# nyrahealth/CrisperWhisper

Measured on AMD Instinct MI355X. Metric: aligned words/s (RTF alongside), CrisperWhisper large-v3 geometry, 30 s chunks, full mel->encoder->decoder->DTW->words path, higher is better.
Workload: dtype bf16

## Files before the change

crisperwhisper_amd/_native.py:

```python
from __future__ import annotations

import ctypes as C
import os

_HERE = os.path.dirname(os.path.abspath(__file__))
LIB_PATH = os.environ.get("CW_LIB_PATH") or os.path.join(_HERE, "libcrisperwhisper.so")

CW_DTYPE_F32, CW_DTYPE_BF16, CW_DTYPE_F16 = 0, 1, 2
N_SAMPLES, N_FRAMES, N_CTX = 480000, 3000, 1500
STAGES = ("mel", "encoder", "cross_kv", "decode", "timestamps")
ALIGN_HEADS_MAX_BYTES = 8 << 30


class NativeLibraryError(RuntimeError):
    pass


class ModelDesc(C.Structure):
    _fields_ = [(n, C.c_int32) for n in (
        "d_model", "n_heads", "ffn_dim", "enc_layers", "dec_layers", "n_mels", "vocab_size",
        "max_target_positions", "median_filter_width", "dtype", "max_batch", "n_align")] + [
        ("align_layers", C.POINTER(C.c_int32)), ("align_heads", C.POINTER(C.c_int32))]


# ... 136 lines not shown
    "cw_test_cross_attention": (_I, [_P, _I, _I, _I, _I, _P, _P, _P, _I, _P, _P, _P, _P]),
    "cw_test_cross_attention_fused": (_I, [_P, _I, _I, _I, _I, _P, _P, _P, _P, _P, _I, _P, _P, _I, _P, _P, _P, _P]),
    "cw_test_fold": (_I, [_P, C.POINTER(FoldArgs)]),
    "cw_test_gemv_stack": (_I, [_P, C.POINTER(GemvStackArgs)]),
    "cw_test_gemv_epi": (_I, [_P, C.POINTER(GemvEpiArgs)]),
    "cw_test_self_attention": (_I, [_P, _I, _I, _I, _I, _P, _P, _P, _P, _I, _P, _I, _I, _I, _I, _P, _P, _P]),
    "cw_test_beam_state": (_I, [_P, _I, _P, _P, _P]),
    "cw_test_prefill_gemm": (_I, [_P, _I, _I, _I, _I, _P, _P, _P, _P]),
    "cw_test_prefill_attention": (_I, [_P, _I, _I, _I, _I, _I, _I, _I, _P, _P, _P, _P]),
    "cw_test_prefill_align_attention": (_I, [_P, _I, _I, _I, _I, _I, _I, _P, _P, _P, _P, _P]),
    "cw_test_score_head": (_I, [_P, _I, _I, _I, _P, _P, _P, _P, _P, _P, _P, _P]),
    "cw_time_score_head": (_I, [_P, _I, _I, _I, _P]),
    "cw_test_beam_topk": (_I, [_P, _I, _P, _P, _I, _I, _I, _I, _P, _P]),
    "cw_test_beam_x": (_I, [_P, _I, _P]),
    "cw_test_sample": (_I, [_P, _I, _P, _P, _I, _I, _I, _I, _P]),
    "cw_test_sample_seeded": (_I, [_P, _I, _P, _P, _I, _I, _I, _I, C.c_float, C.c_uint64, _P, _P]),
    "cw_test_sample_logprobs": (_I, [_P, _I, _P, _P, _I, _I, _I, _I, C.c_float, C.c_uint64, _P, _P, _P, _P]),
    "cw_test_sample_top_logprobs": (_I, [_P, _I, _P, _P, _I, _I, _I, _I, C.c_float, C.c_uint64, _P, _P, _I, _P, _P, _P, _P]),
    "cw_test_sample_biased": (_I, [_P, _I, _P, _P, _I, _I, _I, _I, C.c_float, C.c_uint64, _P, _P, _I, _I, _P, _P, _P, _P, _P, _P, _P, _P]),
    "cw_stage_times": (_I, [_P, _P, _P, _I]),
    "cw_time_kernel": (_I, [_P, _I, _I, _I, _P, _P]),
    "cw_time_decode_stage": (_I, [_P, _I, _I, _I, _P, _P, _P, _P]),
    "cw_decode_stage_name": (C.c_char_p, [_I]),
    "cw_handoff_fallbacks": (_I, [_P]),
    "cw_handoff_resumes": (_I, [_P]),
    "cw_decode_stage_launches": (_I, [_P, _I]),
}

_lib = None

# ... 27 lines not shown
```

crisperwhisper_amd/csrc/elementwise.hip:

```cpp
#include "common.h"
#include "kernels.h"
#include <stdlib.h>

namespace CW_NS {

template <typename T>
__global__ __launch_bounds__(256) void layernorm_kernel(const float* __restrict__ x, const float* __restrict__ g,
                                                        const float* __restrict__ b, T* __restrict__ out, int rows,
                                                        int d) {
    const int lane = threadIdx.x & 63;
    const int row = blockIdx.x * 4 + (threadIdx.x >> 6);
    if (row >= rows) return;
    const float* xr = x + (size_t)row * d;
    T* o = out + (size_t)row * d;
    if (d <= 2048) {
        float4 v[8];
        float s = 0.f;
#pragma unroll
        for (int c = 0; c < 8; ++c) {
            const int k = (lane + 64 * c) * 4;
            v[c] = (k < d) ? *(const float4*)(xr + k) : make_float4(0.f, 0.f, 0.f, 0.f);
            s += (v[c].x + v[c].y) + (v[c].z + v[c].w);
        }
        const float mean = wave_sum(s) / (float)d;
// ... 196 lines not shown
    if (L < 1 || L > SB_MAX_LEN || L > t) return false;
    bool ok = true;
    for (int k = 0; k < L - 1; ++k) ok &= (ids[t - L + 1 + k] == tab[SB_TOK + o + k]);
    return ok;
}
__device__ inline float seq_bias_of(const int* __restrict__ tab, int tok, const int* __restrict__ ids, int t) {
    const int n = min(tab[SB_SLICE + SAMPLE_NS], SB_MAX_SEQ);
    int lo = 0, hi = n;
    while (lo < hi) { const int mid = (lo + hi) >> 1; if (tab[SB_LAST + mid] < tok) lo = mid + 1; else hi = mid; }
    float sum = 0.f;
    for (int e = lo; e < n && tab[SB_LAST + e] == tok; ++e)
        if (seq_bias_applies(tab, e, ids, t)) sum = __fadd_rn(sum, __int_as_float(tab[SB_VAL + e]));
    return sum;
}
#define SAMPLE_THREADS 256
template <bool TOPK, bool BIAS>
__global__ __launch_bounds__(256) void sample_partial_kernel(const float* __restrict__ logits, const int* ids_all, const int* cfg, const int* pos,
                                                             const int* last_ts_tok, const unsigned char* __restrict__ mask, int ldv, int ids_stride,
                                                             SampleParams p, SamplePart* __restrict__ part) {
    __shared__ float s_f[64];
    __shared__ int s_i[64];
    const int b = blockIdx.x, sl = blockIdx.y, tid = threadIdx.x, lane = tid & 63, wave = tid >> 6;
    const float* lg = logits + (size_t)b * ldv;
    const int* ids = ids_all + (size_t)b * ids_stride;
    const int n_prompt = cfg[0], min_new_tokens = cfg[1];
    const int t = pos[b] + 1, tb = p.timestamp_begin;
    const int n_gen = t - n_prompt;
    const bool last_ts = n_gen >= 1 && ids[t - 1] >= tb;
    const bool penult_ts = n_gen < 2 || ids[t - 2] >= tb;
    const int last_tok = last_ts_tok[b];
    const int ts_floor = (last_tok >= 0) ? ((last_ts && !penult_ts) ? last_tok : last_tok + 1) : tb;
    const bool at_begin = (n_gen == 0);
    const int ts_cap = (at_begin && p.max_initial_timestamp_index >= 0) ? tb + p.max_initial_timestamp_index : 0x7fffffff;
    const int per4 = ((ldv >> 2) + SAMPLE_NS - 1) / SAMPLE_NS;
    const int lo4 = sl * per4, hi4 = min(ldv >> 2, lo4 + per4);
    const float4* lg4 = (const float4*)lg;
    const uchar4* mk4 = (const uchar4*)mask;
    ArgPair bt = {-INFINITY, 0x7fffffff}, bs = {-INFINITY, 0x7fffffff};
    ArgPair pt = {-INFINITY, 0x7fffffff}, ps = {-INFINITY, 0x7fffffff};
    const float temp = p.samp ? __uint_as_float(p.samp[0]) : 0.f;
    const bool sampling = temp > 0.f;
    unsigned seed_lo = 0, seed_hi = 0, stream_lo = 0, stream_hi = 0;
    if (sampling) { seed_lo = p.samp[1]; seed_hi = p.samp[2]; stream_lo = p.samp[4 + 2 * b]; stream_hi = p.samp[5 + 2 * b]; }
    float sv[4][4]; int nmine = 0;
    float tv[4][4];
    float rm = -INFINITY, rs = 0.f;
    float rv[4][4];
    if (TOPK) {
#pragma unroll
        for (int it = 0; it < 4; ++it)
#pragma unroll
            for (int j = 0; j < 4; ++j) rv[it][j] = -INFINITY;
    }
    __shared__ float4 s_bias4[BIAS ? 1024 : 1];
    if constexpr (BIAS) {
        __shared__ int s_bl[SB_MAX_SEQ];
        __shared__ float s_bv[SB_MAX_SEQ];
        float* s_bias = (float*)s_bias4;
        for (int k = tid; k < per4; k += 256) s_bias4[k] = make_float4(0.f, 0.f, 0.f, 0.f);
        const int* tab = p.seq_bias;
        const int e0 = tab[SB_SLICE + sl], ne = min(tab[SB_SLICE + sl + 1] - e0, SB_MAX_SEQ);
        const bool have = tid < ne && e0 >= 0 && e0 + ne <= SB_MAX_SEQ;
        int mylast = -1;
        float myval = NAN;
        if (have) {
            mylast = tab[SB_LAST + e0 + tid];
            if (seq_bias_applies(tab, e0 + tid, ids, t)) myval = __int_as_float(tab[SB_VAL + e0 + tid]);
        }
        s_bl[tid] = mylast; s_bv[tid] = myval;
        __syncthreads();
        const int rel = mylast - lo4 * 4;
        if (have && rel >= 0 && rel < per4 * 4 && (tid == 0 || s_bl[tid - 1] != mylast)) {
            float sum = 0.f;
            for (int e = tid; e < SB_MAX_SEQ && s_bl[e] == mylast; ++e)
                if (s_bv[e] == s_bv[e]) sum = __fadd_rn(sum, s_bv[e]);
            s_bias[rel] = sum;
        }
        __syncthreads();
    }
    for (int i4 = lo4 + tid, it = 0; i4 < hi4; i4 += 256, ++it) {
        const float4 x = lg4[i4]; const uchar4 mk = mk4[i4];
        const float xs[4] = {x.x, x.y, x.z, x.w};
        float xe[4] = {x.x, x.y, x.z, x.w};
        if constexpr (BIAS) {
            const float4 bb = s_bias4[i4 - lo4];
            xe[0] = __fadd_rn(x.x, bb.x); xe[1] = __fadd_rn(x.y, bb.y); xe[2] = __fadd_rn(x.z, bb.z); xe[3] = __fadd_rn(x.w, bb.w);
        }
        const unsigned char ms[4] = {mk.x, mk.y, mk.z, mk.w};
        unsigned rnd[4] = {0u, 0u, 0u, 0u};
        if (sampling) philox4x32_10((unsigned)i4, (unsigned)t, stream_lo, stream_hi, seed_lo, seed_hi, rnd);
#pragma unroll
        for (int j = 0; j < 4; ++j) {
            const int v = i4 * 4 + j;
            float val = -INFINITY;
            if (v < p.V) {
                bool dead = (ms[j] & 1) || (at_begin && (ms[j] & 2));
                dead |= (v == p.eos && n_gen < min_new_tokens);
                if (last_ts) dead |= penult_ts ? (v >= tb) : (v < p.eos);
                dead |= (v >= tb && v < ts_floor);
                if (at_begin) dead |= (v < tb) || (v > ts_cap);
                if (!dead) val = xe[j];
                ArgPair c = {val, v};
                if (v < tb) bt = arg_better(bt, c); else bs = arg_better(bs, c);
                if (sampling && !dead) {
                    ArgPair q = {__fadd_rn(__fdiv_rn(val, temp), gumbel_from_bits(rnd[j])), v};
                    if (v < tb) pt = arg_better(pt, q); else ps = arg_better(ps, q);
                }
            }
            if (it < 4) { sv[it][j] = (v >= tb && v < p.V) ? val : -INFINITY; tv[it][j] = (v < tb) ? val : -INFINITY; }
            if (TOPK && it < 4) rv[it][j] = (v < p.V && xs[j] > -INFINITY) ? xs[j] : -INFINITY;
        }
        if (p.tok_lp) {
            float gm = -INFINITY;
#pragma unroll
            for (int j = 0; j < 4; ++j) if (i4 * 4 + j < p.V) gm = fmaxf(gm, xs[j]);
            if (gm > rm) { rs *= expf(rm - gm); rm = gm; }
            if (rm > -INFINITY) {
#pragma unroll
                for (int j = 0; j < 4; ++j) if (i4 * 4 + j < p.V) rs += expf(xs[j] - rm);
            }
        }
        nmine = it + 1;
    }
    bt = wave_argmax(bt);
    bs = wave_argmax(bs);
    if (lane == 0) { s_f[wave] = bt.v; s_i[wave] = bt.i; s_f[32 + wave] = bs.v; s_i[32 + wave] = bs.i; }
    __syncthreads();
    bt = {-INFINITY, 0x7fffffff}; bs = {-INFINITY, 0x7fffffff};
    for (int w = 0; w < 4; ++w) {
        bt = arg_better(bt, ArgPair{s_f[w], s_i[w]});
        bs = arg_better(bs, ArgPair{s_f[32 + w], s_i[32 + w]});
    }
    float acc = 0.f;
    if (bs.v > -INFINITY) {
        for (int it = 0; it < nmine && it < 4; ++it)
#pragma unroll
            for (int j = 0; j < 4; ++j) if (sv[it][j] > -INFINITY) acc += expf(sv[it][j] - bs.v);
    }
    __syncthreads();
    acc = block_sum(acc, s_f);
    float acc_t = 0.f;
    if (p.lp_sum) {
        if (bt.v > -INFINITY) {
            for (int it = 0; it < nmine && it < 4; ++it)
#pragma unroll
                for (int j = 0; j < 4; ++j) if (tv[it][j] > -INFINITY) acc_t += expf(tv[it][j] - bt.v);
        }
        __syncthreads();
        acc_t = block_sum(acc_t, s_f);
    }
    float raw_m = -INFINITY, raw_s = 0.f;
    if (p.tok_lp) {
        __syncthreads();
        raw_m = block_max(rm, s_f);
        __syncthreads();
        raw_s = block_sum(rm > -INFINITY ? rs * expf(rm - raw_m) : 0.f, s_f);
    }
    if (TOPK) {
        __shared__ float s_tf[8];
        __shared__ int s_ti[8];
        TopPair* rec = (TopPair*)p.top_part + ((size_t)b * SAMPLE_NS + sl) * CW_TOP_LOGPROBS_MAX;
        ArgPair prev = {INFINITY, -1};
        for (int r = 0; r < p.top_k; ++r) {
            ArgPair c = {-INFINITY, 0x7fffffff};
#pragma unroll
            for (int it = 0; it < 4; ++it)
#pragma unroll
                for (int j = 0; j < 4; ++j) {
                    const ArgPair q = {rv[it][j], (lo4 + tid + it * 256) * 4 + j};
                    if (q.v > -INFINITY && arg_after(q, prev)) c = arg_better(c, q);
                }
            c = wave_argmax(c);
            const int h = (r & 1) * 4;
            if (lane == 0) { s_tf[h + wave] = c.v; s_ti[h + wave] = c.i; }
            __syncthreads();
            c = {-INFINITY, 0x7fffffff};
            for (int w = 0; w < 4; ++w) c = arg_better(c, ArgPair{s_tf[h + w], s_ti[h + w]});
            if (tid == 0) { TopPair o; o.v = c.v; o.i = c.i; rec[r] = o; }
            prev = c;
        }
    }
// ... 18 lines not shown
        }
    }
    if (tid == 0) {
        SamplePart o; o.bt_v = bt.v; o.bt_i = bt.i; o.bs_v = bs.v; o.bs_i = bs.i; o.ts_sum = acc; o.pad[0] = acc_t; o.pad[1] = raw_m; o.pad[2] = raw_s;
        part[(size_t)b * SAMPLE_NS + sl] = o;
    }
}

template <typename T, bool TOPK, bool BIAS>
__global__ __launch_bounds__(1024) void sample_kernel(int* ids_all, const int* cfg, int* pos, int* finished, int* last_ts_tok,
                                                       const void* partials, int ids_stride, int timestamp_begin, SampleParams p) {
    __shared__ float s_f[64];
    __shared__ int s_i[64];
    __shared__ int s_tok;
    const int b = blockIdx.x, tid = threadIdx.x, lane = tid & 63, wave = tid >> 6, nw = SAMPLE_THREADS >> 6;
    const float* lg = p.logits + (size_t)b * p.ldv;
    int* ids = ids_all + (size_t)b * ids_stride;
    const int n_prompt = cfg[0], min_new_tokens = cfg[1], max_length = cfg[2], use_forced = cfg[3];
    const int t = pos[b] + 1, tb = timestamp_begin;
    const int n_gen = t - n_prompt;

    const int fin_in = finished[b];
    const bool was_finished = fin_in != 0;
    int forced = (p.forced && use_forced) ? p.forced[(size_t)b * ids_stride + t] : -1;

    const bool last_ts = n_gen >= 1 && ids[t - 1] >= tb;
    const bool penult_ts = n_gen < 2 || ids[t - 2] >= tb;
    const int last_tok = last_ts_tok[b];
    const int ts_floor = (last_tok >= 0) ? ((last_ts && !penult_ts) ? last_tok : last_tok + 1) : tb;
    const bool at_begin = (n_gen == 0);
    const int ts_cap = (at_begin && p.max_initial_timestamp_index >= 0) ? tb + p.max_initial_timestamp_index
                                                                         : 0x7fffffff;
    ArgPair bt = {-INFINITY, 0x7fffffff}, bs = {-INFINITY, 0x7fffffff};
    const SamplePart* pr = (const SamplePart*)partials + (size_t)b * SAMPLE_NS;
    for (int i = 0; i < SAMPLE_NS; ++i) {
        bt = arg_better(bt, ArgPair{pr[i].bt_v, pr[i].bt_i});
        bs = arg_better(bs, ArgPair{pr[i].bs_v, pr[i].bs_i});
    }
    const float M = fmaxf(bt.v, bs.v);
    float acc = 0.f;
    for (int i = 0; i < SAMPLE_NS; ++i)
        if (pr[i].bs_v > -INFINITY) acc += pr[i].ts_sum * expf(pr[i].bs_v - M);

    if (TOPK) {
        if (wave == 0 && !was_finished && n_gen >= 0) {
            float Mr = -INFINITY, Sr = 0.f;
            for (int i = 0; i < SAMPLE_NS; ++i) Mr = fmaxf(Mr, pr[i].pad[1]);
            for (int i = 0; i < SAMPLE_NS; ++i)
                if (pr[i].pad[1] > -INFINITY) Sr += pr[i].pad[2] * expf(pr[i].pad[1] - Mr);
            const float norm = Mr + logf(Sr);
            const TopPair* tp = (const TopPair*)p.top_part + (size_t)b * SAMPLE_NS * CW_TOP_LOGPROBS_MAX;
            const int k = p.top_k;
            const ArgPair none = {-INFINITY, 0x7fffffff};
            const bool have = (lane & (CW_TOP_LOGPROBS_MAX - 1)) < k;
            const ArgPair c0 = have ? ArgPair{tp[lane].v, tp[lane].i} : none;
            const ArgPair c1 = have ? ArgPair{tp[lane + 64].v, tp[lane + 64].i} : none;
            ArgPair prev = {INFINITY, -1}, mine = none;
            for (int r = 0; r < k; ++r) {
                ArgPair c = none;
                if (arg_after(c0, prev)) c = arg_better(c, c0);
                if (arg_after(c1, prev)) c = arg_better(c, c1);
                c = wave_argmax(c);
                if (lane == r) mine = c;
                prev = c;
            }
            if (lane < k) {
                const size_t o = ((size_t)b * ids_stride + t) * CW_TOP_LOGPROBS_MAX + lane;
                const bool ok = mine.v > -INFINITY;
                p.top_id[o] = ok ? mine.i : -1;
                p.top_lp[o] = ok ? mine.v - norm : NAN;
            }
        }
    }
    if (tid == 0) {
        bool force_ts = (acc > 0.f) && (logf(acc) > bt.v - M);
        int choice;
        if (force_ts || !(bt.v > -INFINITY)) choice = bs.i;
        else choice = arg_better(bt, bs).i;
        const float temp = p.samp ? __uint_as_float(p.samp[0]) : 0.f;
        if (temp > 0.f) {
            ArgPair pt = {-INFINITY, 0x7fffffff}, ps = {-INFINITY, 0x7fffffff};
            const SamplePert* pp = (const SamplePert*)p.pert + (size_t)b * SAMPLE_NS;
            for (int i = 0; i < SAMPLE_NS; ++i) {
                pt = arg_better(pt, ArgPair{pp[i].pt_v, pp[i].pt_i});
                ps = arg_better(ps, ArgPair{pp[i].ps_v, pp[i].ps_i});
            }
            choice = force_ts ? ps.i : arg_better(pt, ps).i;
        }
        if (!(M > -INFINITY) || choice < 0 || choice >= p.V) choice = 0;
        if (p.argmax_trace) p.argmax_trace[(size_t)b * ids_stride + t] = choice;
        int tok = (forced >= 0) ? forced : choice;
        if (p.lp_sum && !was_finished && n_gen >= 0) {
            float st = 0.f;
            for (int i = 0; i < SAMPLE_NS; ++i)
                if (pr[i].bt_v > -INFINITY) st += pr[i].pad[0] * expf(pr[i].bt_v - M);
            const float tot = acc + (force_ts ? 0.f : st);
            if (tot > 0.f && tok >= 0 && tok < p.V) {
                float xt = lg[tok];
                if constexpr (BIAS) xt = __fadd_rn(xt, seq_bias_of(p.seq_bias, tok, ids, t));
                p.lp_sum[b] += xt - (M + logf(tot));
                p.lp_cnt[b] += 1;
            }
        }
        if (p.tok_lp && !was_finished && n_gen >= 0 && tok >= 0 && tok < p.V) {
            float Mr = -INFINITY, Sr = 0.f;
            for (int i = 0; i < SAMPLE_NS; ++i) Mr = fmaxf(Mr, pr[i].pad[1]);
            for (int i = 0; i < SAMPLE_NS; ++i)
                if (pr[i].pad[1] > -INFINITY) Sr += pr[i].pad[2] * expf(pr[i].pad[1] - Mr);
            p.tok_lp[(size_t)b * ids_stride + t] = lg[tok] - (Mr + logf(Sr));
        }
        if (was_finished) tok = p.pad;
        if (fin_in != 2) ids[t] = tok;
        if (tok >= tb && n_gen >= 0) last_ts_tok[b] = tok;
        int fin = was_finished ? fin_in : ((n_gen >= 0 && tok == p.eos) || (t + 1 >= max_length));
        finished[b] = fin;
        if (!fin) atomicAdd(p.n_unfinished, 1);
        s_tok = tok;
        pos[b] = t;
    }
    __syncthreads();
    const int tok = s_tok;
    if (p.x_out && t < max_length) {
        const T* e = (const T*)p.embed + (size_t)tok * p.d;
        const float* pe = p.pos_embed + (size_t)t * p.d;
        for (int k = tid; k < p.d; k += SAMPLE_THREADS) {
            const float v = Act<T>::ld(e + k) + pe[k];
            p.x_out[(size_t)b * p.d + k] = sizeof(T) == 2 ? resid_grid(v) : v;
        }
    }
}

template <typename T>
__global__ __launch_bounds__(1024) void beam_topk_kernel(SampleParams p, int n_cand, float* __restrict__ cand_val,
                                                         int* __restrict__ cand_id) {
    __shared__ float s_f[64];
    __shared__ int s_i[64];
    const int b = blockIdx.x, tid = threadIdx.x, lane = tid & 63, wave = tid >> 6, nw = blockDim.x >> 6;
    const float* lg = p.logits + (size_t)b * p.ldv;
    const int* ids = p.ids + (size_t)b * p.ids_stride;
    const int n_prompt = p.cfg[0], min_new_tokens = p.cfg[1];
// ... 298 lines not shown
}

template <bool TOPK, bool BIAS>
static void launch_sample_t(const SampleParams& p, hipStream_t st) {
    hipLaunchKernelGGL((sample_partial_kernel<TOPK, BIAS>), dim3(p.B, SAMPLE_NS), dim3(256), 0, st, p.logits, (const int*)p.ids, p.cfg,
                       (const int*)p.pos, (const int*)p.last_ts_tok, p.mask, p.ldv, p.ids_stride, p, (SamplePart*)p.partials);
    if (p.embed_bf16)
        hipLaunchKernelGGL((sample_kernel<bf16_t, TOPK, BIAS>), dim3(p.B), dim3(SAMPLE_THREADS), 0, st, p.ids, p.cfg, p.pos, p.finished,
                           p.last_ts_tok, p.partials, p.ids_stride, p.timestamp_begin, p);
    else
        hipLaunchKernelGGL((sample_kernel<float, TOPK, BIAS>), dim3(p.B), dim3(SAMPLE_THREADS), 0, st, p.ids, p.cfg, p.pos, p.finished,
                           p.last_ts_tok, p.partials, p.ids_stride, p.timestamp_begin, p);
}
int cw_launch_sample(const SampleParams& p, hipStream_t st) {
    static_assert(SAMPLE_NS == 16 && SB_OFF > SB_SLICE + SAMPLE_NS, "the sequence_bias table holds one range per sampler slice");
    if (!p.partials || (p.ldv >> 2) > SAMPLE_NS * 1024 || (p.ldv & 3)) return CW_ERR_INVALID;
    const bool bias = p.seq_bias != nullptr;
    if (p.top_k != 0) {
        if (p.top_k < 0 || p.top_k > CW_TOP_LOGPROBS_MAX || !p.top_part || !p.top_id || !p.top_lp || !p.tok_lp) return CW_ERR_INVALID;
        if (bias) launch_sample_t<true, true>(p, st); else launch_sample_t<true, false>(p, st);
        return CW_OK;
    }
    if (bias) launch_sample_t<false, true>(p, st); else launch_sample_t<false, false>(p, st);
    return CW_OK;
}

}
```

crisperwhisper_amd/csrc/engine.hip:

```cpp
#include <chrono>
#include <hip/hip_runtime.h>
#include <stdarg.h>
#include <stdlib.h>
#include <string.h>
#include <set>
#include <string>
#include <vector>
#include <functional>
#include <algorithm>

#include "../../include/crisperwhisper.h"
#include "kernels.h"

static thread_local char g_err[512] = "";

#define KD(c, fn, ...) ((c)->f16 ? cw_f16::fn(__VA_ARGS__) : cw_bf16::fn(__VA_ARGS__))

#define CW_MAX_DEC_STAGES 24
enum DecStageKind { DST_OTHER = 0, DST_QKV_SELF, DST_QKV, DST_SELF_ATTN, DST_O_PROJ, DST_STACK, DST_STACK_CROSS, DST_CROSS_Q, DST_CROSS_ATTN,
                    DST_CROSS_O, DST_FC1, DST_FC2, DST_MLP_PAIR, DST_MLP_CHAIN, DST_N };
static const char* const kDecStageName[DST_N] = {
    "other (A/B path)", "LayerNorm + q/k/v projection + self-attention (qkv_self_kernel)", "LayerNorm + q/k/v projection + cache append",
    "self-attention", "self-attention out-projection", "fused out-projection + cross-query stage (gemv_stack_kernel)",
    "fused stage + cross-attention (dec_layer_a_kernel)", "LayerNorm + cross-attention query projection", "cross-attention",
// ... 4639 lines not shown
    if (er != hipSuccess) return fail(c, CW_ERR_HIP, "test_beam_topk: %s", hipGetErrorString(er));
    HIPCHK(c, hipMemcpy(cand_val, c->d_cand_val, (size_t)Bm * 64 * 4, hipMemcpyDeviceToHost));
    HIPCHK(c, hipMemcpy(cand_id, c->d_cand_id, (size_t)Bm * 64 * 4, hipMemcpyDeviceToHost));
    return CW_OK;
}

int32_t cw_test_beam_x(cw_ctx* c, int32_t rows, float* x) {
    if (rows < 1 || rows > c->Bm || !x) return fail(c, CW_ERR_INVALID, "test_beam_x: rows=%d", rows);
    HIPCHK(c, hipStreamSynchronize(c->st));
    HIPCHK(c, hipMemcpy(x, c->dx, (size_t)rows * c->d.d_model * 4, hipMemcpyDeviceToHost));
    return CW_OK;
}

static int test_sample(cw_ctx* c, int32_t nb, const float* logits, const int32_t* ids, int32_t t, int32_t n_prompt,
                       int32_t min_new_tokens, int32_t max_length, int32_t* choice_out, const int32_t* forced_tok = nullptr,
                       float* lp_out = nullptr, int32_t* top_id_out = nullptr, float* top_lp_out = nullptr);
int32_t cw_test_sample(cw_ctx* c, int32_t nb, const float* logits, const int32_t* ids, int32_t t, int32_t n_prompt,
                       int32_t min_new_tokens, int32_t max_length, int32_t* choice_out) {
    return test_sample(c, nb, logits, ids, t, n_prompt, min_new_tokens, max_length, choice_out);
}
int32_t cw_test_sample_seeded(cw_ctx* c, int32_t nb, const float* logits, const int32_t* ids, int32_t t, int32_t n_prompt,
                              int32_t min_new_tokens, int32_t max_length, float temperature, uint64_t seed,
                              const uint64_t* row_streams, int32_t* choice_out) {
    if (!logits || !ids || !choice_out) return fail(c, CW_ERR_INVALID, "test_sample_seeded: null argument");
    if (nb < 1 || nb > c->Bm || nb > 64) return fail(c, CW_ERR_INVALID, "test_sample_seeded: nb=%d outside 1 .. %d", nb, c->Bm < 64 ? c->Bm : 64);
    if (max_length <= n_prompt || max_length > c->d.max_target_positions || min_new_tokens < 0)
        return fail(c, CW_ERR_INVALID, "test_sample_seeded: max_length=%d / min_new_tokens=%d out of range", max_length, min_new_tokens);
    if (temperature > 0.f && !row_streams) return fail(c, CW_ERR_INVALID, "test_sample_seeded: a positive temperature needs row_streams");
    const std::vector<unsigned int> keep = c->samp_host;
    CWCHK(c, write_sampling(c, temperature, seed, row_streams, nb, "test_sample_seeded"));
    const int r = test_sample(c, nb, logits, ids, t, n_prompt, min_new_tokens, max_length, choice_out);
    HIPCHK(c, hipStreamSynchronize(c->st));
    HIPCHK(c, hipMemcpy(c->d_samp, keep.data(), keep.size() * 4, hipMemcpyHostToDevice));
    c->samp_host = keep;
// ... 66 lines not shown
    HIPCHK(c, hipMemset(c->d_lp_cnt, 0, (size_t)c->Bm * 4));
    const int r = cw_test_sample_top_logprobs(c, nb, logits, ids, t, n_prompt, min_new_tokens, max_length, temperature, seed, row_streams,
                                              forced_tok, k, choice_out, lp_out, top_id_out, top_lp_out);
    c->score_tokens = keep_score;
    int r2 = CW_OK;
    if (r == CW_OK) {
        hipError_t e = hipMemcpy(proc_lp_out, c->d_lp_sum, (size_t)nb * 4, hipMemcpyDeviceToHost);
        if (e != hipSuccess) r2 = fail(c, CW_ERR_HIP, "test_sample_biased: %s", hipGetErrorString(e));
    }
    drop_step_graphs(c);
    CWCHK(c, seq_bias_install(c, keep, keep_n));
    return r != CW_OK ? r : r2;
}
static int test_sample(cw_ctx* c, int32_t nb, const float* logits, const int32_t* ids, int32_t t, int32_t n_prompt,
                       int32_t min_new_tokens, int32_t max_length, int32_t* choice_out, const int32_t* forced_tok, float* lp_out,
                       int32_t* top_id_out, float* top_lp_out) {
    const int V = c->d.vocab_size, TGT = c->d.max_target_positions;
    if (!c->gen_set) return fail(c, CW_ERR_STATE, "cw_set_generation not called");
    if (nb < 1 || nb > c->Bm || t < n_prompt || t < 1 || t >= TGT || n_prompt < 1) return fail(c, CW_ERR_INVALID, "test_sample: bad args");
    const int tb = c->gen.no_timestamps_token_id + 1;
    std::vector<int> hid((size_t)nb * TGT, c->gen.pad_token_id), last(nb, -1), posv(64, t - 1);
    for (int b = 0; b < nb; ++b)
        for (int k = 0; k < t; ++k) {
            const int tok = ids[(size_t)b * t + k];
            if (tok < 0 || tok >= V) return fail(c, CW_ERR_INVALID, "test_sample: token %d out of range", tok);
            hid[(size_t)b * TGT + k] = tok;
            if (k >= n_prompt && tok >= tb) last[b] = tok;
        }
    HIPCHK(c, hipMemcpy(c->d_ids, hid.data(), hid.size() * 4, hipMemcpyHostToDevice));
    HIPCHK(c, hipMemcpy(c->d_last_ts, last.data(), nb * 4, hipMemcpyHostToDevice));
    HIPCHK(c, hipMemcpy(c->d_pos, posv.data(), 64 * 4, hipMemcpyHostToDevice));
    HIPCHK(c, hipMemset(c->d_finished, 0, nb * 4));
    HIPCHK(c, hipMemset(c->d_argmax, 0xff, (size_t)nb * TGT * 4));
    if (forced_tok) {
        std::vector<int> fr((size_t)nb * TGT, -1);
        for (int b = 0; b < nb; ++b) fr[(size_t)b * TGT + t] = forced_tok[b];
        HIPCHK(c, hipMemcpy(c->d_forced, fr.data(), fr.size() * 4, hipMemcpyHostToDevice));
    }
    if (lp_out) HIPCHK(c, hipMemset(c->d_tok_lp, 0xff, (size_t)nb * TGT * 4));
    if (top_id_out) {
        HIPCHK(c, hipMemset(c->d_top_id, 0xff, (size_t)nb * TGT * CW_TOP_LOGPROBS_MAX * 4));
        HIPCHK(c, hipMemset(c->d_top_lp, 0xff, (size_t)nb * TGT * CW_TOP_LOGPROBS_MAX * 4));
    }
    const int cfg[4] = {n_prompt, min_new_tokens, max_length, forced_tok ? 1 : 0};
    HIPCHK(c, hipMemcpy(c->d_cfg, cfg, sizeof(cfg), hipMemcpyHostToDevice));
    HIPCHK(c, hipMemcpy2D(c->dlogits, (size_t)c->Vpad * 4, logits, (size_t)V * 4, (size_t)V * 4, nb, hipMemcpyHostToDevice));
    const int n_padcol = c->Vpad - V;
// ... 197 lines not shown
```

crisperwhisper_amd/engine.py:

```python
from __future__ import annotations

import ctypes as C
import dataclasses
from typing import Dict, List, Optional, Sequence

import numpy as np

from . import _native as N

_GemvEpiArgs = N.GemvEpiArgs


def _ptr(a: Optional[np.ndarray]):
    return None if a is None else a.ctypes.data_as(C.c_void_p)


def _i32(x) -> np.ndarray:
    return np.ascontiguousarray(np.asarray(x, dtype=np.int32))


@dataclasses.dataclass
class ModelSpec:
    d_model: int
    n_heads: int
# ... 921 lines not shown
    def test_beam_x(self, rows: int) -> np.ndarray:
        x = np.zeros((int(rows), self.spec.d_model), np.float32)
        self._chk(self.lib.cw_test_beam_x(self.ctx, int(rows), _ptr(x)))
        return x

    def test_sample(self, logits: np.ndarray, ids: np.ndarray, n_prompt: int, min_new_tokens: int = 0,
                    max_length: Optional[int] = None) -> np.ndarray:
        lg = np.ascontiguousarray(logits, np.float32)
        ids = _i32(ids)
        nb, t = ids.shape
        out = np.zeros(nb, np.int32)
        self._chk(self.lib.cw_test_sample(self.ctx, nb, _ptr(lg), _ptr(ids), t, int(n_prompt), int(min_new_tokens),
                                          int(max_length or self.spec.max_target_positions), _ptr(out)))
        return out

    def test_sample_seeded(self, logits: np.ndarray, ids: np.ndarray, n_prompt: int, temperature: float, seed: int,
                           row_streams, min_new_tokens: int = 0, max_length: Optional[int] = None) -> np.ndarray:
        lg = np.ascontiguousarray(logits, np.float32)
        ids = _i32(ids)
        nb, t = ids.shape
        if lg.shape != (nb, self.spec.vocab_size):
            raise ValueError(f"logits must be [{nb}][{self.spec.vocab_size}], got {lg.shape}")
        rs = None if row_streams is None else np.ascontiguousarray(row_streams, dtype=np.uint64)
        if rs is not None and rs.shape != (nb,):
            raise ValueError(f"row_streams must hold one id per row ({nb}), got shape {rs.shape}")
        out = np.zeros(nb, np.int32)
        self._chk(self.lib.cw_test_sample_seeded(self.ctx, nb, _ptr(lg), _ptr(ids), t, int(n_prompt), int(min_new_tokens),
                                                 int(max_length or self.spec.max_target_positions), float(temperature),
                                                 int(seed) & (2 ** 64 - 1), _ptr(rs), _ptr(out)))
        return out
# ... 102 lines not shown
```

include/crisperwhisper.h:

```cpp
#ifndef CRISPERWHISPER_H
#define CRISPERWHISPER_H

#include <stdint.h>

#ifdef __cplusplus
extern "C" {
#endif

typedef struct cw_ctx cw_ctx;

#define CW_DTYPE_F32 0
#define CW_DTYPE_BF16 1
#define CW_DTYPE_F16 2

#define CW_N_SAMPLES 480000
#define CW_N_FRAMES 3000
#define CW_N_CTX 1500

typedef struct {
    int32_t d_model, n_heads, ffn_dim, enc_layers, dec_layers, n_mels, vocab_size;
    int32_t max_target_positions;
    int32_t median_filter_width;
    int32_t dtype;
    int32_t max_batch;
// ... 277 lines not shown
    float* cvec;
    int32_t* nt;
    int32_t* frag_tail_ok;
} cw_test_gemv_epi_args;
int32_t cw_test_gemv_epi(cw_ctx* ctx, const cw_test_gemv_epi_args* args);
int32_t cw_test_self_attention(cw_ctx* ctx, int32_t B, int32_t H, int32_t cap, int32_t kv_div, const float* q, const float* k,
                               const float* v, const int32_t* pos, int32_t n_keys, const int32_t* anc, int32_t short_hist,
                               int32_t out_frag, int32_t align_head, int32_t align_rows, float* out, float* align,
                               int32_t* frag_tail_ok);
int32_t cw_test_beam_state(cw_ctx* ctx, int32_t rows, int32_t* ids, int32_t* anc, int32_t* pos);
int32_t cw_test_beam_topk(cw_ctx* ctx, int32_t nb, const float* logits, const int32_t* ids, int32_t t, int32_t n_prompt,
                          int32_t min_new_tokens, int32_t n_cand, float* cand_val, int32_t* cand_id);
int32_t cw_test_beam_x(cw_ctx* ctx, int32_t rows, float* x);
int32_t cw_test_sample(cw_ctx* ctx, int32_t nb, const float* logits, const int32_t* ids, int32_t t, int32_t n_prompt,
                       int32_t min_new_tokens, int32_t max_length, int32_t* choice_out);
int32_t cw_test_sample_seeded(cw_ctx* ctx, int32_t nb, const float* logits, const int32_t* ids, int32_t t, int32_t n_prompt,
                              int32_t min_new_tokens, int32_t max_length, float temperature, uint64_t seed,
                              const uint64_t* row_streams, int32_t* choice_out);
int32_t cw_test_sample_logprobs(cw_ctx* ctx, int32_t nb, const float* logits, const int32_t* ids, int32_t t, int32_t n_prompt,
                                int32_t min_new_tokens, int32_t max_length, float temperature, uint64_t seed,
                                const uint64_t* row_streams, const int32_t* forced_tok, int32_t* choice_out, float* lp_out);
int32_t cw_test_sample_top_logprobs(cw_ctx* ctx, int32_t nb, const float* logits, const int32_t* ids, int32_t t, int32_t n_prompt,
                                    int32_t min_new_tokens, int32_t max_length, float temperature, uint64_t seed,
                                    const uint64_t* row_streams, const int32_t* forced_tok, int32_t k, int32_t* choice_out,
                                    float* lp_out, int32_t* top_id_out, float* top_lp_out);
int32_t cw_test_sample_biased(cw_ctx* ctx, int32_t nb, const float* logits, const int32_t* ids, int32_t t, int32_t n_prompt,
                              int32_t min_new_tokens, int32_t max_length, float temperature, uint64_t seed,
                              const uint64_t* row_streams, const int32_t* forced_tok, int32_t k, int32_t n_seq,
                              const int32_t* seq_tokens, const int32_t* seq_lengths, const float* seq_bias, int32_t* choice_out,
                              float* lp_out, int32_t* top_id_out, float* top_lp_out, float* proc_lp_out);
// ... 21 lines not shown
```

Before: 791.8.

## Front-load logit loads and wave-parallelize partial reduction in sampler kernels

The stage-1 sampler kernel now issues all four float4 logit and mask loads up front, together with the cfg/pos/last_ts scalar loads, behind a scheduling barrier. This hides global-memory latency before the per-token masking logic runs, and the sampling/logprob extras move to a separate second pass. The stage-2 finalize kernel reads the per-slice partials across lanes and reduces them with wave_argmax and readlane, replacing serial loops over SAMPLE_NS. It also prefetches the position embedding, forced token and temperature early. A test entry point for a full sample step is added as well. The cost is more register pressure and a second pass over the logits when sampling or token logprobs are on.

```diff
diff --git a/crisperwhisper_amd/_native.py b/crisperwhisper_amd/_native.py
--- a/crisperwhisper_amd/_native.py
+++ b/crisperwhisper_amd/_native.py
@@ -174,6 +174,7 @@
     "cw_test_beam_topk": (_I, [_P, _I, _P, _P, _I, _I, _I, _I, _P, _P]),
     "cw_test_beam_x": (_I, [_P, _I, _P]),
     "cw_test_sample": (_I, [_P, _I, _P, _P, _I, _I, _I, _I, _P]),
+    "cw_test_sample_step": (_I, [_P, _I, _P, _P, _I, _I, _I, _I, _P, _P, _P, _P, _P, _P, _P, _P]),
     "cw_test_sample_seeded": (_I, [_P, _I, _P, _P, _I, _I, _I, _I, C.c_float, C.c_uint64, _P, _P]),
     "cw_test_sample_logprobs": (_I, [_P, _I, _P, _P, _I, _I, _I, _I, C.c_float, C.c_uint64, _P, _P, _P, _P]),
     "cw_test_sample_top_logprobs": (_I, [_P, _I, _P, _P, _I, _I, _I, _I, C.c_float, C.c_uint64, _P, _P, _I, _P, _P, _P, _P]),
diff --git a/crisperwhisper_amd/csrc/elementwise.hip b/crisperwhisper_amd/csrc/elementwise.hip
--- a/crisperwhisper_amd/csrc/elementwise.hip
+++ b/crisperwhisper_amd/csrc/elementwise.hip
@@ -234,6 +234,13 @@
     return sum;
 }
 #define SAMPLE_THREADS 256
+__device__ inline int opaque_zero_vgpr() {
+    int z;
+    asm("v_mov_b32 %0, 0" : "=v"(z));
+    return z;
+}
+#define SAMPLE_XTRIPS 5
+#define SAMPLE_TRIPS 4
 template <bool TOPK, bool BIAS>
 __global__ __launch_bounds__(256) void sample_partial_kernel(const float* __restrict__ logits, const int* ids_all, const int* cfg, const int* pos,
                                                              const int* last_ts_tok, const unsigned char* __restrict__ mask, int ldv, int ids_stride,
@@ -241,34 +248,45 @@
     __shared__ float s_f[64];
     __shared__ int s_i[64];
     const int b = blockIdx.x, sl = blockIdx.y, tid = threadIdx.x, lane = tid & 63, wave = tid >> 6;
-    const float* lg = logits + (size_t)b * ldv;
+    const int nv4 = ldv >> 2;
+    const int per4 = (nv4 + SAMPLE_NS - 1) / SAMPLE_NS;
+    const int lo4 = sl * per4, hi4 = min(nv4, lo4 + per4);
+    const float4* lg4 = (const float4*)(logits + (size_t)b * ldv);
+    const uchar4* mk4 = (const uchar4*)mask;
+    const int vz = opaque_zero_vgpr();
+    const int cfg0_q = cfg[vz], cfg1_q = cfg[vz + 1], pos_q = pos[b + vz], last_q = last_ts_tok[b + vz];
+#define SAMPLE_REQ(n) const int ic##n = min(lo4 + tid + n * 256, nv4 - 1); const float4 xq##n = lg4[ic##n]; const uchar4 mq##n = mk4[ic##n]
+    SAMPLE_REQ(0); SAMPLE_REQ(1); SAMPLE_REQ(2); SAMPLE_REQ(3);
+#undef SAMPLE_REQ
+    __builtin_amdgcn_sched_barrier(0);
+    const int n_prompt = __builtin_amdgcn_readfirstlane(cfg0_q), min_new_tokens = __builtin_amdgcn_readfirstlane(cfg1_q);
+    const int pos_b = __builtin_amdgcn_readfirstlane(pos_q), last_tok = __builtin_amdgcn_readfirstlane(last_q);
     const int* ids = ids_all + (size_t)b * ids_stride;
-    const int n_prompt = cfg[0], min_new_tokens = cfg[1];
-    const int t = pos[b] + 1, tb = p.timestamp_begin;
+    const int tb = p.timestamp_begin;
+    const unsigned int* sp = p.samp ? p.samp : (const unsigned int*)cfg;
+    const int t = pos_b + 1;
     const int n_gen = t - n_prompt;
-    const bool last_ts = n_gen >= 1 && ids[t - 1] >= tb;
-    const bool penult_ts = n_gen < 2 || ids[t - 2] >= tb;
-    const int last_tok = last_ts_tok[b];
+    const int id1 = ids[max(min(t - 1, ids_stride - 1), 0)], id2 = ids[max(min(t - 2, ids_stride - 1), 0)];
+    const unsigned s0 = sp[0];
+    __builtin_amdgcn_sched_barrier(0);
+    const bool last_ts = n_gen >= 1 && id1 >= tb;
+    const bool penult_ts = n_gen < 2 || id2 >= tb;
     const int ts_floor = (last_tok >= 0) ? ((last_ts && !penult_ts) ? last_tok : last_tok + 1) : tb;
     const bool at_begin = (n_gen == 0);
     const int ts_cap = (at_begin && p.max_initial_timestamp_index >= 0) ? tb + p.max_initial_timestamp_index : 0x7fffffff;
-    const int per4 = ((ldv >> 2) + SAMPLE_NS - 1) / SAMPLE_NS;
-    const int lo4 = sl * per4, hi4 = min(ldv >> 2, lo4 + per4);
-    const float4* lg4 = (const float4*)lg;
-    const uchar4* mk4 = (const uchar4*)mask;
     ArgPair bt = {-INFINITY, 0x7fffffff}, bs = {-INFINITY, 0x7fffffff};
     ArgPair pt = {-INFINITY, 0x7fffffff}, ps = {-INFINITY, 0x7fffffff};
-    const float temp = p.samp ? __uint_as_float(p.samp[0]) : 0.f;
+    const float temp = p.samp ? __uint_as_float(s0) : 0.f;
     const bool sampling = temp > 0.f;
     unsigned seed_lo = 0, seed_hi = 0, stream_lo = 0, stream_hi = 0;
     if (sampling) { seed_lo = p.samp[1]; seed_hi = p.samp[2]; stream_lo = p.samp[4 + 2 * b]; stream_hi = p.samp[5 + 2 * b]; }
-    float sv[4][4]; int nmine = 0;
-    float tv[4][4];
+    float sv[SAMPLE_TRIPS][4]; int nmine = 0;
+    float tv[SAMPLE_TRIPS][4];
     float rm = -INFINITY, rs = 0.f;
-    float rv[4][4];
+    float rv[SAMPLE_TRIPS][4];
     if (TOPK) {
 #pragma unroll
-        for (int it = 0; it < 4; ++it)
+        for (int it = 0; it < SAMPLE_TRIPS; ++it)
 #pragma unroll
             for (int j = 0; j < 4; ++j) rv[it][j] = -INFINITY;
     }
@@ -298,8 +316,7 @@
         }
         __syncthreads();
     }
-    for (int i4 = lo4 + tid, it = 0; i4 < hi4; i4 += 256, ++it) {
-        const float4 x = lg4[i4]; const uchar4 mk = mk4[i4];
+    auto trip = [&](const float4 x, const uchar4 mk, const int i4, const int it, const bool live, const bool core, const bool extras) {
         const float xs[4] = {x.x, x.y, x.z, x.w};
         float xe[4] = {x.x, x.y, x.z, x.w};
         if constexpr (BIAS) {
@@ -308,12 +325,12 @@
         }
         const unsigned char ms[4] = {mk.x, mk.y, mk.z, mk.w};
         unsigned rnd[4] = {0u, 0u, 0u, 0u};
-        if (sampling) philox4x32_10((unsigned)i4, (unsigned)t, stream_lo, stream_hi, seed_lo, seed_hi, rnd);
+        if (extras && sampling) philox4x32_10((unsigned)i4, (unsigned)t, stream_lo, stream_hi, seed_lo, seed_hi, rnd);
 #pragma unroll
         for (int j = 0; j < 4; ++j) {
             const int v = i4 * 4 + j;
             float val = -INFINITY;
-            if (v < p.V) {
+            if (live && v < p.V) {
                 bool dead = (ms[j] & 1) || (at_begin && (ms[j] & 2));
                 dead |= (v == p.eos && n_gen < min_new_tokens);
                 if (last_ts) dead |= penult_ts ? (v >= tb) : (v < p.eos);
@@ -321,16 +338,16 @@
                 if (at_begin) dead |= (v < tb) || (v > ts_cap);
                 if (!dead) val = xe[j];
                 ArgPair c = {val, v};
-                if (v < tb) bt = arg_better(bt, c); else bs = arg_better(bs, c);
-                if (sampling && !dead) {
+                if (core) { if (v < tb) bt = arg_better(bt, c); else bs = arg_better(bs, c); }
+                if (extras && sampling && !dead) {
                     ArgPair q = {__fadd_rn(__fdiv_rn(val, temp), gumbel_from_bits(rnd[j])), v};
                     if (v < tb) pt = arg_better(pt, q); else ps = arg_better(ps, q);
                 }
             }
-            if (it < 4) { sv[it][j] = (v >= tb && v < p.V) ? val : -INFINITY; tv[it][j] = (v < tb) ? val : -INFINITY; }
-            if (TOPK && it < 4) rv[it][j] = (v < p.V && xs[j] > -INFINITY) ? xs[j] : -INFINITY;
-        }
-        if (p.tok_lp) {
+            if (core && it < SAMPLE_TRIPS) { sv[it][j] = (v >= tb) ? val : -INFINITY; tv[it][j] = (v < tb) ? val : -INFINITY; }
+            if (TOPK && core && it < SAMPLE_TRIPS) rv[it][j] = (live && v < p.V && xs[j] > -INFINITY) ? xs[j] : -INFINITY;
+        }
+        if (extras && p.tok_lp) {
             float gm = -INFINITY;
 #pragma unroll
             for (int j = 0; j < 4; ++j) if (i4 * 4 + j < p.V) gm = fmaxf(gm, xs[j]);
@@ -340,8 +357,20 @@
                 for (int j = 0; j < 4; ++j) if (i4 * 4 + j < p.V) rs += expf(xs[j] - rm);
             }
         }
-        nmine = it + 1;
-    }
+        if (core && live) nmine = it + 1;
+    };
+    trip(xq0, mq0, lo4 + tid, 0, lo4 + tid < hi4, true, false);
+    trip(xq1, mq1, lo4 + tid + 256, 1, lo4 + tid + 256 < hi4, true, false);
+    trip(xq2, mq2, lo4 + tid + 512, 2, lo4 + tid + 512 < hi4, true, false);
+    trip(xq3, mq3, lo4 + tid + 768, 3, lo4 + tid + 768 < hi4, true, false);
+    if (sampling || p.tok_lp) {
+#pragma unroll 1
+        for (int it = 0; it < SAMPLE_TRIPS; ++it) {
+            const int i4 = lo4 + tid + it * 256;
+            if (i4 < hi4) trip(lg4[i4], mk4[i4], i4, SAMPLE_TRIPS, true, false, true);
+        }
+    }
+    for (int i4 = lo4 + tid + SAMPLE_TRIPS * 256; i4 < hi4; i4 += 256) trip(lg4[i4], mk4[i4], i4, SAMPLE_TRIPS, true, true, true);
     bt = wave_argmax(bt);
     bs = wave_argmax(bs);
     if (lane == 0) { s_f[wave] = bt.v; s_i[wave] = bt.i; s_f[32 + wave] = bs.v; s_i[32 + wave] = bs.i; }
@@ -353,7 +382,7 @@
     }
     float acc = 0.f;
     if (bs.v > -INFINITY) {
-        for (int it = 0; it < nmine && it < 4; ++it)
+        for (int it = 0; it < nmine && it < SAMPLE_TRIPS; ++it)
 #pragma unroll
             for (int j = 0; j < 4; ++j) if (sv[it][j] > -INFINITY) acc += expf(sv[it][j] - bs.v);
     }
@@ -362,7 +391,7 @@
     float acc_t = 0.f;
     if (p.lp_sum) {
         if (bt.v > -INFINITY) {
-            for (int it = 0; it < nmine && it < 4; ++it)
+            for (int it = 0; it < nmine && it < SAMPLE_TRIPS; ++it)
 #pragma unroll
                 for (int j = 0; j < 4; ++j) if (tv[it][j] > -INFINITY) acc_t += expf(tv[it][j] - bt.v);
         }
@@ -384,7 +413,7 @@
         for (int r = 0; r < p.top_k; ++r) {
             ArgPair c = {-INFINITY, 0x7fffffff};
 #pragma unroll
-            for (int it = 0; it < 4; ++it)
+            for (int it = 0; it < SAMPLE_TRIPS; ++it)
 #pragma unroll
                 for (int j = 0; j < 4; ++j) {
                     const ArgPair q = {rv[it][j], (lo4 + tid + it * 256) * 4 + j};
@@ -433,47 +462,75 @@
     __shared__ int s_i[64];
     __shared__ int s_tok;
     const int b = blockIdx.x, tid = threadIdx.x, lane = tid & 63, wave = tid >> 6, nw = SAMPLE_THREADS >> 6;
+    const SamplePart* pr = (const SamplePart*)partials + (size_t)b * SAMPLE_NS;
+    const int rl = lane & (SAMPLE_NS - 1);
+    const float4 ra = ((const float4*)(pr + rl))[0];
+    const float4 rb = ((const float4*)(pr + rl))[1];
+    __builtin_amdgcn_sched_barrier(0);
+    int* ids = ids_all + (size_t)b * ids_stride;
+    const int n_prompt = cfg[0], max_length = cfg[2], use_forced = cfg[3];
+    const int pos_b = pos[b];
+    const int fin_in = finished[b];
     const float* lg = p.logits + (size_t)b * p.ldv;
-    int* ids = ids_all + (size_t)b * ids_stride;
-    const int n_prompt = cfg[0], min_new_tokens = cfg[1], max_length = cfg[2], use_forced = cfg[3];
-    const int t = pos[b] + 1, tb = timestamp_begin;
+    const int tb = timestamp_begin;
+    asm volatile("" ::"s"(n_prompt), "s"(max_length), "s"(use_forced), "s"(pos_b), "s"(fin_in), "s"(p.V), "s"(p.eos), "s"(p.pad),
+                 "s"(p.argmax_trace), "s"(p.n_unfinished), "s"(p.lp_sum), "s"(p.tok_lp), "s"(p.embed));
+    __builtin_amdgcn_sched_barrier(0);
+    const int t = pos_b + 1;
     const int n_gen = t - n_prompt;
-
-    const int fin_in = finished[b];
     const bool was_finished = fin_in != 0;
-    int forced = (p.forced && use_forced) ? p.forced[(size_t)b * ids_stride + t] : -1;
-
-    const bool last_ts = n_gen >= 1 && ids[t - 1] >= tb;
-    const bool penult_ts = n_gen < 2 || ids[t - 2] >= tb;
-    const int last_tok = last_ts_tok[b];
-    const int ts_floor = (last_tok >= 0) ? ((last_ts && !penult_ts) ? last_tok : last_tok + 1) : tb;
-    const bool at_begin = (n_gen == 0);
-    const int ts_cap = (at_begin && p.max_initial_timestamp_index >= 0) ? tb + p.max_initial_timestamp_index
-                                                                         : 0x7fffffff;
-    ArgPair bt = {-INFINITY, 0x7fffffff}, bs = {-INFINITY, 0x7fffffff};
-    const SamplePart* pr = (const SamplePart*)partials + (size_t)b * SAMPLE_NS;
-    for (int i = 0; i < SAMPLE_NS; ++i) {
-        bt = arg_better(bt, ArgPair{pr[i].bt_v, pr[i].bt_i});
-        bs = arg_better(bs, ArgPair{pr[i].bs_v, pr[i].bs_i});
-    }
+    const bool embed_next = p.x_out && t < max_length;
+    const float* pe = embed_next ? p.pos_embed + (size_t)t * p.d : (const float*)pr;
+    float peq[SAMPLE_XTRIPS];
+#pragma unroll
+    for (int i = 0; i < SAMPLE_XTRIPS; ++i) peq[i] = pe[embed_next ? min(tid + i * SAMPLE_THREADS, p.d - 1) : 0];
+    const bool have_forced = p.forced && use_forced;
+    const int forced_w = *(have_forced ? p.forced + (size_t)b * ids_stride + t : cfg);
+    const int forced = have_forced ? forced_w : -1;
+    const unsigned temp_w = *(p.samp ? p.samp : (const unsigned int*)cfg);
+    const float temp = p.samp ? __uint_as_float(temp_w) : 0.f;
+    const float4 rp = *(p.pert ? (const float4*)p.pert + (size_t)b * SAMPLE_NS + rl : (const float4*)(pr + rl));
+    ArgPair c0 = {-INFINITY, 0x7fffffff}, c1 = {-INFINITY, 0x7fffffff};
+    if constexpr (TOPK) {
+        const TopPair* tp = (const TopPair*)p.top_part + (size_t)b * SAMPLE_NS * CW_TOP_LOGPROBS_MAX;
+        const TopPair t0 = tp[lane], t1 = tp[lane + 64];
+        c0 = ArgPair{t0.v, t0.i}; c1 = ArgPair{t1.v, t1.i};
+    }
+    asm volatile("" ::"s"(forced_w), "s"(temp_w));
+    __builtin_amdgcn_sched_barrier(0);
+    const ArgPair bt = wave_argmax(ArgPair{ra.x, __float_as_int(ra.y)}), bs = wave_argmax(ArgPair{ra.z, __float_as_int(ra.w)});
+    const ArgPair pt = wave_argmax(ArgPair{rp.x, __float_as_int(rp.y)}), ps = wave_argmax(ArgPair{rp.z, __float_as_int(rp.w)});
     const float M = fmaxf(bt.v, bs.v);
+#define SAMPLE_REC(x, i) __int_as_float(__builtin_amdgcn_readlane(__float_as_int(x), i))
+    const float e_bs = expf(ra.z - M), e_bt = expf(ra.x - M);
     float acc = 0.f;
+#pragma unroll
     for (int i = 0; i < SAMPLE_NS; ++i)
-        if (pr[i].bs_v > -INFINITY) acc += pr[i].ts_sum * expf(pr[i].bs_v - M);
+        if (SAMPLE_REC(ra.z, i) > -INFINITY) acc += SAMPLE_REC(rb.x, i) * SAMPLE_REC(e_bs, i);
+    float st = 0.f;
+    if (p.lp_sum) {
+#pragma unroll
+        for (int i = 0; i < SAMPLE_NS; ++i)
+            if (SAMPLE_REC(ra.x, i) > -INFINITY) st += SAMPLE_REC(rb.y, i) * SAMPLE_REC(e_bt, i);
+    }
+    float Mr = -INFINITY, Sr = 0.f;
+    if (p.tok_lp) {
+#pragma unroll
+        for (int i = 0; i < SAMPLE_NS; ++i) Mr = fmaxf(Mr, SAMPLE_REC(rb.z, i));
+        const float e_r = expf(rb.z - Mr);
+#pragma unroll
+        for (int i = 0; i < SAMPLE_NS; ++i)
+            if (SAMPLE_REC(rb.z, i) > -INFINITY) Sr += SAMPLE_REC(rb.w, i) * SAMPLE_REC(e_r, i);
+    }
+#undef SAMPLE_REC
 
     if (TOPK) {
         if (wave == 0 && !was_finished && n_gen >= 0) {
-            float Mr = -INFINITY, Sr = 0.f;
-            for (int i = 0; i < SAMPLE_NS; ++i) Mr = fmaxf(Mr, pr[i].pad[1]);
-            for (int i = 0; i < SAMPLE_NS; ++i)
-                if (pr[i].pad[1] > -INFINITY) Sr += pr[i].pad[2] * expf(pr[i].pad[1] - Mr);
             const float norm = Mr + logf(Sr);
-            const TopPair* tp = (const TopPair*)p.top_part + (size_t)b * SAMPLE_NS * CW_TOP_LOGPROBS_MAX;
             const int k = p.top_k;
             const ArgPair none = {-INFINITY, 0x7fffffff};
             const bool have = (lane & (CW_TOP_LOGPROBS_MAX - 1)) < k;
-            const ArgPair c0 = have ? ArgPair{tp[lane].v, tp[lane].i} : none;
-            const ArgPair c1 = have ? ArgPair{tp[lane + 64].v, tp[lane + 64].i} : none;
+            if (!have) c0 = c1 = none;
             ArgPair prev = {INFINITY, -1}, mine = none;
             for (int r = 0; r < k; ++r) {
                 ArgPair c = none;
@@ -496,23 +553,11 @@
         int choice;
         if (force_ts || !(bt.v > -INFINITY)) choice = bs.i;
         else choice = arg_better(bt, bs).i;
-        const float temp = p.samp ? __uint_as_float(p.samp[0]) : 0.f;
-        if (temp > 0.f) {
-            ArgPair pt = {-INFINITY, 0x7fffffff}, ps = {-INFINITY, 0x7fffffff};
-            const SamplePert* pp = (const SamplePert*)p.pert + (size_t)b * SAMPLE_NS;
-            for (int i = 0; i < SAMPLE_NS; ++i) {
-                pt = arg_better(pt, ArgPair{pp[i].pt_v, pp[i].pt_i});
-                ps = arg_better(ps, ArgPair{pp[i].ps_v, pp[i].ps_i});
-            }
-            choice = force_ts ? ps.i : arg_better(pt, ps).i;
-        }
+        if (temp > 0.f) choice = force_ts ? ps.i : arg_better(pt, ps).i;
         if (!(M > -INFINITY) || choice < 0 || choice >= p.V) choice = 0;
         if (p.argmax_trace) p.argmax_trace[(size_t)b * ids_stride + t] = choice;
         int tok = (forced >= 0) ? forced : choice;
         if (p.lp_sum && !was_finished && n_gen >= 0) {
-            float st = 0.f;
-            for (int i = 0; i < SAMPLE_NS; ++i)
-                if (pr[i].bt_v > -INFINITY) st += pr[i].pad[0] * expf(pr[i].bt_v - M);
             const float tot = acc + (force_ts ? 0.f : st);
             if (tot > 0.f && tok >= 0 && tok < p.V) {
                 float xt = lg[tok];
@@ -522,10 +567,6 @@
             }
         }
         if (p.tok_lp && !was_finished && n_gen >= 0 && tok >= 0 && tok < p.V) {
-            float Mr = -INFINITY, Sr = 0.f;
-            for (int i = 0; i < SAMPLE_NS; ++i) Mr = fmaxf(Mr, pr[i].pad[1]);
-            for (int i = 0; i < SAMPLE_NS; ++i)
-                if (pr[i].pad[1] > -INFINITY) Sr += pr[i].pad[2] * expf(pr[i].pad[1] - Mr);
             p.tok_lp[(size_t)b * ids_stride + t] = lg[tok] - (Mr + logf(Sr));
         }
         if (was_finished) tok = p.pad;
@@ -539,10 +580,18 @@
     }
     __syncthreads();
     const int tok = s_tok;
-    if (p.x_out && t < max_length) {
+    if (embed_next) {
         const T* e = (const T*)p.embed + (size_t)tok * p.d;
-        const float* pe = p.pos_embed + (size_t)t * p.d;
-        for (int k = tid; k < p.d; k += SAMPLE_THREADS) {
+        float eq[SAMPLE_XTRIPS];
+#pragma unroll
+        for (int i = 0; i < SAMPLE_XTRIPS; ++i) eq[i] = Act<T>::ld(e + min(tid + i * SAMPLE_THREADS, p.d - 1));
+#pragma unroll
+        for (int i = 0; i < SAMPLE_XTRIPS; ++i) {
+            const int k = tid + i * SAMPLE_THREADS;
+            const float v = eq[i] + peq[i];
+            if (k < p.d) p.x_out[(size_t)b * p.d + k] = sizeof(T) == 2 ? resid_grid(v) : v;
+        }
+        for (int k = tid + SAMPLE_XTRIPS * SAMPLE_THREADS; k < p.d; k += SAMPLE_THREADS) {
             const float v = Act<T>::ld(e + k) + pe[k];
             p.x_out[(size_t)b * p.d + k] = sizeof(T) == 2 ? resid_grid(v) : v;
         }
@@ -871,7 +920,8 @@
 }
 int cw_launch_sample(const SampleParams& p, hipStream_t st) {
     static_assert(SAMPLE_NS == 16 && SB_OFF > SB_SLICE + SAMPLE_NS, "the sequence_bias table holds one range per sampler slice");
-    if (!p.partials || (p.ldv >> 2) > SAMPLE_NS * 1024 || (p.ldv & 3)) return CW_ERR_INVALID;
+    static_assert(SAMPLE_TRIPS == 4 && SAMPLE_TRIPS * 256 == 1024, "a stage-1 block holds its slice in SAMPLE_TRIPS trips of 256 threads");
+    if (!p.partials || p.ldv < 4 || (p.ldv >> 2) > SAMPLE_NS * SAMPLE_TRIPS * 256 || (p.ldv & 3)) return CW_ERR_INVALID;
     const bool bias = p.seq_bias != nullptr;
     if (p.top_k != 0) {
         if (p.top_k < 0 || p.top_k > CW_TOP_LOGPROBS_MAX || !p.top_part || !p.top_id || !p.top_lp || !p.tok_lp) return CW_ERR_INVALID;
diff --git a/crisperwhisper_amd/csrc/engine.hip b/crisperwhisper_amd/csrc/engine.hip
--- a/crisperwhisper_amd/csrc/engine.hip
+++ b/crisperwhisper_amd/csrc/engine.hip
@@ -4677,10 +4677,35 @@
 
 static int test_sample(cw_ctx* c, int32_t nb, const float* logits, const int32_t* ids, int32_t t, int32_t n_prompt,
                        int32_t min_new_tokens, int32_t max_length, int32_t* choice_out, const int32_t* forced_tok = nullptr,
-                       float* lp_out = nullptr, int32_t* top_id_out = nullptr, float* top_lp_out = nullptr);
+                       float* lp_out = nullptr, int32_t* top_id_out = nullptr, float* top_lp_out = nullptr,
+                       const int32_t* finished_in = nullptr);
 int32_t cw_test_sample(cw_ctx* c, int32_t nb, const float* logits, const int32_t* ids, int32_t t, int32_t n_prompt,
                        int32_t min_new_tokens, int32_t max_length, int32_t* choice_out) {
     return test_sample(c, nb, logits, ids, t, n_prompt, min_new_tokens, max_length, choice_out);
+}
+int32_t cw_test_sample_step(cw_ctx* c, int32_t nb, const float* logits, const int32_t* ids, int32_t t, int32_t n_prompt,
+                            int32_t min_new_tokens, int32_t max_length, const int32_t* forced_tok, const int32_t* finished_in,
+                            int32_t* choice_out, int32_t* tok_out, int32_t* last_ts_out, int32_t* finished_out, int32_t* pos_out,
+                            int32_t* n_unfinished_out) {
+    if (!logits || !ids || !choice_out || !tok_out || !last_ts_out || !finished_out || !pos_out || !n_unfinished_out)
+        return fail(c, CW_ERR_INVALID, "test_sample_step: null argument");
+    if (nb < 1 || nb > c->Bm || nb > 64) return fail(c, CW_ERR_INVALID, "test_sample_step: nb=%d outside 1 .. %d", nb, c->Bm < 64 ? c->Bm : 64);
+    if (max_length <= n_prompt || max_length > c->d.max_target_positions || min_new_tokens < 0)
+        return fail(c, CW_ERR_INVALID, "test_sample_step: max_length=%d / min_new_tokens=%d out of range", max_length, min_new_tokens);
+    for (int b = 0; b < nb; ++b) {
+        if (forced_tok && forced_tok[b] >= c->d.vocab_size) return fail(c, CW_ERR_INVALID, "test_sample_step: forced token %d out of range", forced_tok[b]);
+        if (finished_in && (finished_in[b] < 0 || finished_in[b] > 2)) return fail(c, CW_ERR_INVALID, "test_sample_step: finished_in[%d]=%d", b, finished_in[b]);
+    }
+    CWCHK(c, test_sample(c, nb, logits, ids, t, n_prompt, min_new_tokens, max_length, choice_out, forced_tok, nullptr, nullptr, nullptr, finished_in));
+    const int TGT = c->d.max_target_positions;
+    std::vector<int> hid((size_t)nb * TGT);
+    HIPCHK(c, hipMemcpy(hid.data(), c->d_ids, hid.size() * 4, hipMemcpyDeviceToHost));
+    for (int b = 0; b < nb; ++b) tok_out[b] = hid[(size_t)b * TGT + t];
+    HIPCHK(c, hipMemcpy(last_ts_out, c->d_last_ts, (size_t)nb * 4, hipMemcpyDeviceToHost));
+    HIPCHK(c, hipMemcpy(finished_out, c->d_finished, (size_t)nb * 4, hipMemcpyDeviceToHost));
+    HIPCHK(c, hipMemcpy(pos_out, c->d_pos, (size_t)nb * 4, hipMemcpyDeviceToHost));
+    HIPCHK(c, hipMemcpy(n_unfinished_out, c->d_nunf, 4, hipMemcpyDeviceToHost));
+    return CW_OK;
 }
 int32_t cw_test_sample_seeded(cw_ctx* c, int32_t nb, const float* logits, const int32_t* ids, int32_t t, int32_t n_prompt,
                               int32_t min_new_tokens, int32_t max_length, float temperature, uint64_t seed,
@@ -4777,7 +4802,7 @@
 }
 static int test_sample(cw_ctx* c, int32_t nb, const float* logits, const int32_t* ids, int32_t t, int32_t n_prompt,
                        int32_t min_new_tokens, int32_t max_length, int32_t* choice_out, const int32_t* forced_tok, float* lp_out,
-                       int32_t* top_id_out, float* top_lp_out) {
+                       int32_t* top_id_out, float* top_lp_out, const int32_t* finished_in) {
     const int V = c->d.vocab_size, TGT = c->d.max_target_positions;
     if (!c->gen_set) return fail(c, CW_ERR_STATE, "cw_set_generation not called");
     if (nb < 1 || nb > c->Bm || t < n_prompt || t < 1 || t >= TGT || n_prompt < 1) return fail(c, CW_ERR_INVALID, "test_sample: bad args");
@@ -4793,7 +4818,8 @@
     HIPCHK(c, hipMemcpy(c->d_ids, hid.data(), hid.size() * 4, hipMemcpyHostToDevice));
     HIPCHK(c, hipMemcpy(c->d_last_ts, last.data(), nb * 4, hipMemcpyHostToDevice));
     HIPCHK(c, hipMemcpy(c->d_pos, posv.data(), 64 * 4, hipMemcpyHostToDevice));
-    HIPCHK(c, hipMemset(c->d_finished, 0, nb * 4));
+    if (finished_in) HIPCHK(c, hipMemcpy(c->d_finished, finished_in, (size_t)nb * 4, hipMemcpyHostToDevice));
+    else HIPCHK(c, hipMemset(c->d_finished, 0, nb * 4));
     HIPCHK(c, hipMemset(c->d_argmax, 0xff, (size_t)nb * TGT * 4));
     if (forced_tok) {
         std::vector<int> fr((size_t)nb * TGT, -1);
diff --git a/crisperwhisper_amd/engine.py b/crisperwhisper_amd/engine.py
--- a/crisperwhisper_amd/engine.py
+++ b/crisperwhisper_amd/engine.py
@@ -959,6 +959,28 @@
                                           int(max_length or self.spec.max_target_positions), _ptr(out)))
         return out
 
+    def test_sample_step(self, logits: np.ndarray, ids: np.ndarray, n_prompt: int, min_new_tokens: int = 0,
+                         max_length: Optional[int] = None, forced=None, finished=None) -> dict:
+        lg = np.ascontiguousarray(logits, np.float32)
+        ids = _i32(ids)
+        nb, t = ids.shape
+        if lg.shape != (nb, self.spec.vocab_size):
+            raise ValueError(f"logits must be [{nb}][{self.spec.vocab_size}], got {lg.shape}")
+        fr = None if forced is None else _i32(forced)
+        fi = None if finished is None else _i32(finished)
+        for name, a in (("forced", fr), ("finished", fi)):
+            if a is not None and a.shape != (nb,):
+                raise ValueError(f"{name} must hold one value per row ({nb}), got shape {a.shape}")
+        out = {k: np.zeros(nb, np.int32) for k in ("choice", "tok", "last_ts", "finished", "pos")}
+        nunf = np.zeros(1, np.int32)
+        self._chk(self.lib.cw_test_sample_step(self.ctx, nb, _ptr(lg), _ptr(ids), t, int(n_prompt), int(min_new_tokens),
+                                               int(max_length or self.spec.max_target_positions), _ptr(fr), _ptr(fi),
+                                               _ptr(out["choice"]), _ptr(out["tok"]), _ptr(out["last_ts"]), _ptr(out["finished"]),
+                                               _ptr(out["pos"]), _ptr(nunf)))
+        out["n_unfinished"] = int(nunf[0])
+        out["x"] = self.test_beam_x(nb)
+        return out
+
     def test_sample_seeded(self, logits: np.ndarray, ids: np.ndarray, n_prompt: int, temperature: float, seed: int,
                            row_streams, min_new_tokens: int = 0, max_length: Optional[int] = None) -> np.ndarray:
         lg = np.ascontiguousarray(logits, np.float32)
diff --git a/include/crisperwhisper.h b/include/crisperwhisper.h
--- a/include/crisperwhisper.h
+++ b/include/crisperwhisper.h
@@ -315,6 +315,10 @@
 int32_t cw_test_beam_x(cw_ctx* ctx, int32_t rows, float* x);
 int32_t cw_test_sample(cw_ctx* ctx, int32_t nb, const float* logits, const int32_t* ids, int32_t t, int32_t n_prompt,
                        int32_t min_new_tokens, int32_t max_length, int32_t* choice_out);
+int32_t cw_test_sample_step(cw_ctx* ctx, int32_t nb, const float* logits, const int32_t* ids, int32_t t, int32_t n_prompt,
+                            int32_t min_new_tokens, int32_t max_length, const int32_t* forced_tok, const int32_t* finished_in,
+                            int32_t* choice_out, int32_t* tok_out, int32_t* last_ts_out, int32_t* finished_out, int32_t* pos_out,
+                            int32_t* n_unfinished_out);
 int32_t cw_test_sample_seeded(cw_ctx* ctx, int32_t nb, const float* logits, const int32_t* ids, int32_t t, int32_t n_prompt,
                               int32_t min_new_tokens, int32_t max_length, float temperature, uint64_t seed,
                               const uint64_t* row_streams, int32_t* choice_out);
```

Measured after the change: 794.4 (median of 2 runs). About the same (+0.3%).
